# carpedkm/disentangled-subject-to-vid

Hardware: AMD Instinct MI355X
Metric: denoise steps/sec (CogVideoX-5B, 49f 720x480; one step = CFG-pair transformer forward + CFG + scheduler step) (higher is better)
Workload: dtype bf16

## Files before the change

### disentangled-subject-to-vid_amd/csrc/elementwise.hip

```cpp
#define S2V_HOST
#include "common.h"
#include "kernels.h"
#include <cstdlib>
#include <type_traits>

#define LN_MAX_FLOATS 64
template <typename T, int NR>
__device__ __forceinline__ void row_load(const T* x, int D, int lane, float* v) {
    constexpr int VN = Vec16<T>::N;
    const int chunks = D / VN;
#pragma unroll
    for (int i = 0; i < NR; ++i) {
        const int c = lane + 64 * i;
        const bool ok = c < chunks;
        Vec16<T>::ld(x + (ok ? c : 0) * VN, v + i * VN);
#pragma unroll
        for (int e = 0; e < VN; ++e) v[i * VN + e] = ok ? v[i * VN + e] : 0.f;
    }
}
template <typename T, int NR>
__device__ __forceinline__ void row_layernorm(float* v, int D, int lane, const T* w, const T* b, float eps) {
    constexpr int VN = Vec16<T>::N;
    const int chunks = D / VN;
    float s = 0.f;
#pragma unroll
    for (int i = 0; i < NR * VN; ++i) s += v[i];
    const float mean = wave_sum(s) / (float)D;
    float q = 0.f;
#pragma unroll
    for (int i = 0; i < NR; ++i) {
        const bool ok = lane + 64 * i < chunks;
#pragma unroll
        for (int e = 0; e < VN; ++e) {
            const float d = v[i * VN + e] - mean;
            q += ok ? d * d : 0.f;
        }
    }
    const float var = wave_sum(q) / (float)D;
    const float rstd = 1.0f / sqrtf(var + eps);
#pragma unroll
    for (int i = 0; i < NR; ++i) {
        const int c = lane + 64 * i;
        const bool ok = c < chunks;
        const int cc = ok ? c : 0;
        float wv[VN], bv[VN];
        Vec16<T>::ld(w + cc * VN, wv);
        Vec16<T>::ld(b + cc * VN, bv);
#pragma unroll
        for (int e = 0; e < VN; ++e) v[i * VN + e] = ok ? ET<T>::rnd((v[i * VN + e] - mean) * rstd * wv[e] + bv[e]) : 0.f;
    }
}
template <typename T, int NR>
__device__ __forceinline__ void row_modulate_store(float* v, int D, int lane, const T* shift, const T* scale, T* y) {
    constexpr int VN = Vec16<T>::N;
    const int chunks = D / VN;
#pragma unroll
    for (int i = 0; i < NR; ++i) {
        const int c = lane + 64 * i;
        const bool ok = c < chunks;
        const int cc = ok ? c : 0;
        float sc[VN], sh[VN], o[VN];
        Vec16<T>::ld(scale + cc * VN, sc);
        Vec16<T>::ld(shift + cc * VN, sh);
#pragma unroll
        for (int e = 0; e < VN; ++e) {
            const float s1 = ET<T>::rnd(1.0f + sc[e]);
            const float p = ET<T>::rnd(v[i * VN + e] * s1);
            o[e] = p + sh[e];
        }
        if (ok) Vec16<T>::st(y + c * VN, o);
    }
}
template <int NR>
__device__ __forceinline__ void row_modulate_quant_store(float* v, int D, int lane, const bf16_t* shift, const bf16_t* scale, unsigned char* q,
                                                         float* qscale, bf16_t* y = nullptr ) {
    const int chunks = D / 8;
    float amax = 0.f;
#pragma unroll
    for (int i = 0; i < NR; ++i) {
        const int c = lane + 64 * i;
        const bool ok = c < chunks;
        const int cc = ok ? c : 0;
        float sc[8], sh[8];
        Vec16<bf16_t>::ld(scale + cc * 8, sc);
        Vec16<bf16_t>::ld(shift + cc * 8, sh);
#pragma unroll
        for (int e = 0; e < 8; ++e) {
            const float s1 = ET<bf16_t>::rnd(1.0f + sc[e]);
            const float p = ET<bf16_t>::rnd(v[i * 8 + e] * s1);
            const float o = ok ? ET<bf16_t>::rnd(p + sh[e]) : 0.f;
            v[i * 8 + e] = o;
            amax = fmaxf(amax, fabsf(o));
        }
    }
    amax = wave_max(amax);
    const float sc = amax > 0.f ? amax * (1.0f / 448.0f) : 1.0f;
    const float inv = 1.0f / sc;
    if (lane == 0) *qscale = sc;
#pragma unroll
    for (int i = 0; i < NR; ++i) {
        const int c = lane + 64 * i;
        int w0 = 0, w1 = 0;
        w0 = __builtin_amdgcn_cvt_pk_fp8_f32(v[i * 8 + 0] * inv, v[i * 8 + 1] * inv, w0, false);
        w0 = __builtin_amdgcn_cvt_pk_fp8_f32(v[i * 8 + 2] * inv, v[i * 8 + 3] * inv, w0, true);
        w1 = __builtin_amdgcn_cvt_pk_fp8_f32(v[i * 8 + 4] * inv, v[i * 8 + 5] * inv, w1, false);
        w1 = __builtin_amdgcn_cvt_pk_fp8_f32(v[i * 8 + 6] * inv, v[i * 8 + 7] * inv, w1, true);
        if (c < chunks) *(u32x2*)(q + c * 8) = u32x2{(unsigned)w0, (unsigned)w1};
        if (y != nullptr && c < chunks) Vec16<bf16_t>::st(y + c * 8, v + i * 8);
    }
}
template <typename T, int NR>
struct RowParams { typename Vec16<T>::raw_t w[NR], b[NR], sc[NR], sh[NR]; };
template <typename T, int NR>
__device__ __forceinline__ void row_params(RowParams<T, NR>& p, int D, int lane, const T* w, const T* b, const T* scale, const T* shift) {
    constexpr int VN = Vec16<T>::N;
    const int chunks = D / VN;
#pragma unroll
    for (int i = 0; i < NR; ++i) {
        const int c = lane + 64 * i;
        const int cc = c < chunks ? c : 0;
        p.w[i] = Vec16<T>::ldraw(w + cc * VN);
        p.b[i] = Vec16<T>::ldraw(b + cc * VN);
        p.sc[i] = Vec16<T>::ldraw(scale + cc * VN);
        p.sh[i] = Vec16<T>::ldraw(shift + cc * VN);
    }
    __builtin_amdgcn_sched_barrier(0);
}
template <typename T, int NR>
__device__ __forceinline__ void row_layernorm_p(float* v, int D, int lane, const RowParams<T, NR>& p, float eps) {
    constexpr int VN = Vec16<T>::N;
    const int chunks = D / VN;
    float s = 0.f;
#pragma unroll
    for (int i = 0; i < NR * VN; ++i) s += v[i];
    const float mean = wave_sum(s) / (float)D;
    float q = 0.f;
#pragma unroll
    for (int i = 0; i < NR; ++i) {
        const bool ok = lane + 64 * i < chunks;
#pragma unroll
        for (int e = 0; e < VN; ++e) {
            const float d = v[i * VN + e] - mean;
            q += ok ? d * d : 0.f;
        }
    }
    const float var = wave_sum(q) / (float)D;
    const float rstd = 1.0f / sqrtf(var + eps);
#pragma unroll
    for (int i = 0; i < NR; ++i) {
        const bool ok = lane + 64 * i < chunks;
        float wv[VN], bv[VN];
        Vec16<T>::dec(p.w[i], wv);
        Vec16<T>::dec(p.b[i], bv);
#pragma unroll
        for (int e = 0; e < VN; ++e) v[i * VN + e] = ok ? ET<T>::rnd((v[i * VN + e] - mean) * rstd * wv[e] + bv[e]) : 0.f;
    }
}
template <typename T, int NR>
__device__ __forceinline__ void row_modulate_store_p(float* v, int D, int lane, const RowParams<T, NR>& p, T* y) {
    constexpr int VN = Vec16<T>::N;
    const int chunks = D / VN;
#pragma unroll
    for (int i = 0; i < NR; ++i) {
        const int c = lane + 64 * i;
        float sc[VN], sh[VN], o[VN];
        Vec16<T>::dec(p.sc[i], sc);
        Vec16<T>::dec(p.sh[i], sh);
#pragma unroll
        for (int e = 0; e < VN; ++e) {
            const float s1 = ET<T>::rnd(1.0f + sc[e]);
            const float pr = ET<T>::rnd(v[i * VN + e] * s1);
            o[e] = pr + sh[e];
        }
        if (c < chunks) Vec16<T>::st(y + c * VN, o);
    }
}

template <typename T> static int ln_rounds(int D) {
    const int need = (D / Vec16<T>::N + 63) / 64;
    for (int r : {1, 2, 3, 4, 6, 8, 12, 16})
        if (r >= need) return r;
    return -1;
}
#define S2V_LN_DISPATCH(T, D, ...)                                                   \
    switch (ln_rounds<T>(D)) {                                                        \
        case 1: { constexpr int NR = 1; __VA_ARGS__; } break;                                \
        case 2: { constexpr int NR = 2; __VA_ARGS__; } break;                                \
        case 3: { constexpr int NR = 3; __VA_ARGS__; } break;                                \
        case 4: { constexpr int NR = 4; __VA_ARGS__; } break;                                \
        case 6: { constexpr int NR = 6; __VA_ARGS__; } break;                                \
        case 8: { constexpr int NR = 8; __VA_ARGS__; } break;                                \
        case 12: if constexpr (sizeof(T) == 4) { constexpr int NR = 12; __VA_ARGS__; } break; \
        case 16: if constexpr (sizeof(T) == 4) { constexpr int NR = 16; __VA_ARGS__; } break; \
        default: return s2v_fail(__FILE__, __LINE__, "layer norm: row too long", -1); \
    }

template <typename T, int NR>
__global__ __launch_bounds__(256) void ln_modulate_k(const LnModArgs a) {
    const int lane = threadIdx.x & 63;
    const int row = blockIdx.x * 4 + (threadIdx.x >> 6);
    if (row >= a.B * a.Ntok) return;
    const int b = row / a.Ntok, r = row - b * a.Ntok;
    const bool txt = r < a.text_len;
    const bool ref = a.shift_ref != nullptr && !txt && r < a.text_len + a.ref_len;
    const T* shift = (const T*)(txt ? a.shift_txt : ref ? a.shift_ref : a.shift_vid) + (size_t)b * a.mod_stride;
    const T* scale = (const T*)(txt ? a.scale_txt : ref ? a.scale_ref : a.scale_vid) + (size_t)b * a.mod_stride;
    float v[NR * Vec16<T>::N];
    if constexpr (std::is_same<T, bf16_t>::value) {
        if (a.q8 != nullptr) {
            row_load<T, NR>((const T*)a.x + (size_t)row * a.ldx, a.D, lane, v);
            row_layernorm<T, NR>(v, a.D, lane, (const T*)a.w, (const T*)a.b, a.eps);
            row_modulate_quant_store<NR>(v, a.D, lane, shift, scale, (unsigned char*)a.q8 + (size_t)row * a.D, a.q8_scale + row,
                                         a.q8_keep_y ? (bf16_t*)a.y + (size_t)row * a.ldy : nullptr);
            return;
        }
    }
    typename Vec16<T>::raw_t xr[NR];
    {
        constexpr int VN = Vec16<T>::N;
        const int chunks = a.D / VN;
        const T* x = (const T*)a.x + (size_t)row * a.ldx;
#pragma unroll
        for (int i = 0; i < NR; ++i) xr[i] = Vec16<T>::ldraw(x + (lane + 64 * i < chunks ? lane + 64 * i : 0) * VN);
        RowParams<T, NR> prm;
        row_params<T, NR>(prm, a.D, lane, (const T*)a.w, (const T*)a.b, scale, shift);
#pragma unroll
        for (int i = 0; i < NR; ++i) {
            Vec16<T>::dec(xr[i], v + i * VN);
            const bool ok = lane + 64 * i < chunks;
#pragma unroll
            for (int e = 0; e < VN; ++e) v[i * VN + e] = ok ? v[i * VN + e] : 0.f;
        }
        row_layernorm_p<T, NR>(v, a.D, lane, prm, a.eps);
        row_modulate_store_p<T, NR>(v, a.D, lane, prm, (T*)a.y + (size_t)row * a.ldy);
    }
}
template <typename T, int NR, int RPW>
__global__ __launch_bounds__(256) void ln_modulate_lds_k(const LnModArgs a) {
    extern __shared__ __attribute__((aligned(16))) char ln_smem[];
    constexpr int VN = Vec16<T>::N;
    const int lane = threadIdx.x & 63, wave = threadIdx.x >> 6;
    const int rows = a.B * a.Ntok, r0 = blockIdx.x * (4 * RPW), rl = min(r0 + 4 * RPW, rows) - 1;
    auto params_of = [&](int row, const T*& shift, const T*& scale) {
        const int b = row / a.Ntok, r = row - b * a.Ntok;
        const bool txt = r < a.text_len;
        const bool ref = a.shift_ref != nullptr && !txt && r < a.text_len + a.ref_len;
        shift = (const T*)(txt ? a.shift_txt : ref ? a.shift_ref : a.shift_vid) + (size_t)b * a.mod_stride;
        scale = (const T*)(txt ? a.scale_txt : ref ? a.scale_ref : a.scale_vid) + (size_t)b * a.mod_stride;
    };
    const T *sh0, *sc0, *sh1, *sc1;
    params_of(r0, sh0, sc0);
    params_of(rl, sh1, sc1);
    const bool uniform = sh0 == sh1 && sc0 == sc1;
    T* lw = (T*)ln_smem;
    T *lb = lw + a.D, *lsc = lb + a.D, *lsh = lsc + a.D;
    if (uniform) {
        const int chunks = a.D / VN;
        for (int c = threadIdx.x; c < chunks; c += 256) {
            *(typename Vec16<T>::raw_t*)(lw + c * VN) = Vec16<T>::ldraw((const T*)a.w + c * VN);
            *(typename Vec16<T>::raw_t*)(lb + c * VN) = Vec16<T>::ldraw((const T*)a.b + c * VN);
            *(typename Vec16<T>::raw_t*)(lsc + c * VN) = Vec16<T>::ldraw(sc0 + c * VN);
            *(typename Vec16<T>::raw_t*)(lsh + c * VN) = Vec16<T>::ldraw(sh0 + c * VN);
        }
        __syncthreads();
    }
#pragma unroll 1
    for (int k = 0; k < RPW; ++k) {
        const int row = r0 + k * 4 + wave;
        if (row >= rows) break;
        const T *pw = lw, *pb = lb, *psc = lsc, *psh = lsh;
        if (!uniform) { pw = (const T*)a.w; pb = (const T*)a.b; params_of(row, psh, psc); }
        float v[NR * VN];
        row_load<T, NR>((const T*)a.x + (size_t)row * a.ldx, a.D, lane, v);
        row_layernorm<T, NR>(v, a.D, lane, pw, pb, a.eps);
        if constexpr (std::is_same<T, bf16_t>::value) {
            if (a.q8 != nullptr) {
                row_modulate_quant_store<NR>(v, a.D, lane, psh, psc, (unsigned char*)a.q8 + (size_t)row * a.D, a.q8_scale + row,
                                             a.q8_keep_y ? (bf16_t*)a.y + (size_t)row * a.ldy : nullptr);
                continue;
            }
        }
        row_modulate_store<T, NR>(v, a.D, lane, psh, psc, (T*)a.y + (size_t)row * a.ldy);
    }
}
int launch_ln_modulate(const LnModArgs& a, int dtype, hipStream_t st) {
    S2V_REQUIRE(a.D <= 4096 && a.D % 8 == 0, "ln_modulate: D must be <= 4096 and a multiple of 8");
    S2V_REQUIRE(a.q8 == nullptr || (dtype == S2V_BF16 && a.q8_scale != nullptr), "ln_modulate: the fp8 output needs bf16 rows and a scale vector");
    const int rows = a.B * a.Ntok;
    dim3 grid((rows + 3) / 4);
    int lds_rows = 16384;
#ifdef S2V_DIAG
    if (const char* e = getenv("S2V_LN_LDS_ROWS")) lds_rows = atoi(e);
#endif
    if (dtype == S2V_BF16 && lds_rows > 0 && rows >= lds_rows) {
        constexpr int RPW = 4;
        dim3 g16((rows + 4 * RPW - 1) / (4 * RPW));
        const size_t lds = (size_t)4 * a.D * 2;
        S2V_LN_DISPATCH(bf16_t, a.D, hipLaunchKernelGGL((ln_modulate_lds_k<bf16_t, NR, RPW>), g16, dim3(256), lds, st, a))
        S2V_CHECK_HIP(hipGetLastError());
        return 0;
    }
    if (dtype == S2V_BF16) {
        S2V_LN_DISPATCH(bf16_t, a.D, hipLaunchKernelGGL((ln_modulate_k<bf16_t, NR>), grid, dim3(256), 0, st, a))
    } else if (dtype == S2V_F16) {
        S2V_LN_DISPATCH(f16_t, a.D, hipLaunchKernelGGL((ln_modulate_k<f16_t, NR>), grid, dim3(256), 0, st, a))
    } else {
        S2V_LN_DISPATCH(float, a.D, hipLaunchKernelGGL((ln_modulate_k<float, NR>), grid, dim3(256), 0, st, a))
    }
    S2V_CHECK_HIP(hipGetLastError());
    return 0;
}

template <typename T, int NR>
__global__ __launch_bounds__(256) void tail_norm_k(const TailNormArgs a) {
    const int lane = threadIdx.x & 63;
    const int idx = blockIdx.x * 4 + (threadIdx.x >> 6);
    if (idx >= a.B * a.V) return;
    const int b = idx / a.V, vr = idx - b * a.V;
    const size_t xrow = (size_t)b * a.Ntok + a.row0 + vr;
    float v[NR * Vec16<T>::N];
    row_load<T, NR>((const T*)a.x + xrow * a.ldx, a.D, lane, v);
    row_layernorm<T, NR>(v, a.D, lane, (const T*)a.w1, (const T*)a.b1, a.eps);
    row_layernorm<T, NR>(v, a.D, lane, (const T*)a.w2, (const T*)a.b2, a.eps);
    const T* shift = (const T*)a.shift + (size_t)b * a.mod_stride;
    const T* scale = (const T*)a.scale + (size_t)b * a.mod_stride;
    row_modulate_store<T, NR>(v, a.D, lane, shift, scale, (T*)a.y + (size_t)idx * a.ldy);
}
int launch_tail_norm(const TailNormArgs& a, int dtype, hipStream_t st) {
    S2V_REQUIRE(a.D <= 4096 && a.D % 8 == 0, "tail_norm: D must be <= 4096 and a multiple of 8");
    dim3 grid((a.B * a.V + 3) / 4);
    if (dtype == S2V_BF16) {
        S2V_LN_DISPATCH(bf16_t, a.D, hipLaunchKernelGGL((tail_norm_k<bf16_t, NR>), grid, dim3(256), 0, st, a))
    } else if (dtype == S2V_F16) {
        S2V_LN_DISPATCH(f16_t, a.D, hipLaunchKernelGGL((tail_norm_k<f16_t, NR>), grid, dim3(256), 0, st, a))
    } else {
        S2V_LN_DISPATCH(float, a.D, hipLaunchKernelGGL((tail_norm_k<float, NR>), grid, dim3(256), 0, st, a))
    }
    S2V_CHECK_HIP(hipGetLastError());
    return 0;
}

template <typename T>
__global__ __launch_bounds__(256) void qk_norm_rope_k(const QkNormRopeArgs a) {
    const int D = a.H * 64;
    const int row = blockIdx.x;
    const int t = blockIdx.y * 256 + threadIdx.x;
    if (t >= 2 * a.H * 8) return;
    const int which = t >= a.H * 8;
    const int hh = (t >> 3) - which * a.H;
    const int oct = t & 7;
    T* p = (T*)a.qkv + (size_t)row * a.ld_qkv + which * D + hh * 64 + oct * 8;
    const int r = row % a.Ntok;
    const bool rope = a.cos != nullptr && r >= a.text_len;
    const size_t tab = (size_t)(rope ? r - a.text_len : 0) * 64 + oct * 8;
    float v[8], cs[8], sn[8], wv[8], bv[8];
    if constexpr (sizeof(T) == 2) {
        Vec16<T>::ld(p, v);
    } else {
        Vec16<T>::ld(p, v);
        Vec16<T>::ld(p + 4, v + 4);
    }
    if (a.cos != nullptr) {
        Vec16<float>::ld(a.cos + tab, cs);
        Vec16<float>::ld(a.cos + tab + 4, cs + 4);
        Vec16<float>::ld(a.sin + tab, sn);
        Vec16<float>::ld(a.sin + tab + 4, sn + 4);
    }
    const T* w = (const T*)(which ? a.nk_w : a.nq_w) + oct * 8;
    const T* bb = (const T*)(which ? a.nk_b : a.nq_b) + oct * 8;
    if constexpr (sizeof(T) == 2) {
        Vec16<T>::ld(w, wv);
        Vec16<T>::ld(bb, bv);
    } else {
        Vec16<T>::ld(w, wv);
        Vec16<T>::ld(w + 4, wv + 4);
        Vec16<T>::ld(bb, bv);
        Vec16<T>::ld(bb + 4, bv + 4);
    }
    float s = 0.f;
#pragma unroll
    for (int e = 0; e < 8; ++e) s += v[e];
    s += __shfl_xor(s, 1, 64); s += __shfl_xor(s, 2, 64); s += __shfl_xor(s, 4, 64);
    const float mean = s * (1.0f / 64.0f);
    float q = 0.f;
#pragma unroll
    for (int e = 0; e < 8; ++e) { const float d = v[e] - mean; q += d * d; }
    q += __shfl_xor(q, 1, 64); q += __shfl_xor(q, 2, 64); q += __shfl_xor(q, 4, 64);
    const float rstd = 1.0f / sqrtf(q * (1.0f / 64.0f) + a.eps);
#pragma unroll
    for (int e = 0; e < 8; ++e) v[e] = ET<T>::rnd((v[e] - mean) * rstd * wv[e] + bv[e]);
    if (rope) {
#pragma unroll
        for (int e = 0; e < 8; e += 2) {
            const float x0 = v[e], x1 = v[e + 1];
            v[e] = ET<T>::rnd(x0 * cs[e] + (-x1) * sn[e]);
            v[e + 1] = ET<T>::rnd(x1 * cs[e + 1] + x0 * sn[e + 1]);
        }
    }
    if constexpr (sizeof(T) == 2) {
        Vec16<T>::st(p, v);
    } else {
        Vec16<T>::st(p, v);
        Vec16<T>::st(p + 4, v + 4);
    }
}

__global__ __launch_bounds__(256) void v_amax_k(const bf16_t* qkv, int ld_qkv, int H, int Ntok, unsigned* vamax) {
    const int n0 = blockIdx.x * 64, h = blockIdx.y, b = blockIdx.z;
    const int D = H * 64;
    unsigned m = 0;
    for (int i = threadIdx.x; i < 64 * 8; i += 256) {
        const int n = n0 + (i >> 3), cc = (i & 7) * 8;
        if (n < Ntok) {
            const u32x4 val = *(const u32x4*)(qkv + (size_t)(b * Ntok + n) * ld_qkv + 2 * D + h * 64 + cc);
#pragma unroll
            for (int e = 0; e < 4; ++e) m = max(m, max(val[e] & 0x7fffu, (val[e] >> 16) & 0x7fffu));
        }
    }
#pragma unroll
    for (int o = 32; o > 0; o >>= 1) m = max(m, (unsigned)__shfl_xor((int)m, o, 64));
    if ((threadIdx.x & 63) == 0 && m != 0) atomicMax(vamax + b * H + h, m);
}
__global__ __launch_bounds__(256) void v_transpose_k(const bf16_t* qkv, int ld_qkv, int B, int H, int Ntok, bf16_t* vt,
                                                     int ntok_pad, const unsigned* vamax) {
    __shared__ bf16_t tile[64][64 + 2];
    const int n0 = blockIdx.x * 64, h = blockIdx.y, b = blockIdx.z;
    const int D = H * 64;
    const int tid = threadIdx.x;
    const bool to_f16 = vamax != nullptr;
    const float vscale = to_f16 ? __uint_as_float((unsigned)(127 + vt_f16_shift(vamax[b * H + h])) << 23) : 1.0f;
    for (int i = tid; i < 64 * 8; i += 256) {
        const int rr = i >> 3, cc = (i & 7) * 8;
        const int n = n0 + rr;
        u32x4 val = {0, 0, 0, 0};
        if (n < Ntok) val = *(const u32x4*)(qkv + (size_t)(b * Ntok + n) * ld_qkv + 2 * D + h * 64 + cc);
#pragma unroll
        for (int e = 0; e < 4; ++e) {
            tile[rr][cc + 2 * e] = (bf16_t)(val[e] & 0xffff);
            tile[rr][cc + 2 * e + 1] = (bf16_t)(val[e] >> 16);
        }
    }
    __syncthreads();
    bf16_t* dst = vt + (size_t)(b * H + h) * 64 * ntok_pad;
    for (int i = tid; i < 64 * 64; i += 256) {
        const int d = i >> 6, pos = i & 63;
        const int tok = (pos & ~12) | ((pos & 4) << 1) | ((pos & 8) >> 1);
        if (n0 + tok < Ntok) {
            bf16_t v = tile[tok][d];
            if (to_f16) {
                float f = __uint_as_float((unsigned)v << 16) * vscale;
                f = f != f ? f : fminf(fmaxf(f, -65504.0f), 65504.0f);
                v = __builtin_bit_cast(unsigned short, (_Float16)f);
            }
            dst[(size_t)d * ntok_pad + n0 + pos] = v;
        }
        else if (n0 + pos < ntok_pad) dst[(size_t)d * ntok_pad + n0 + pos] = 0;
    }
}

__global__ __launch_bounds__(256) void qk_quant_mx_k(const bf16_t* qkv, int ld_qkv, int H, int Ntok, int ntok_pad, float q_prescale,
                                                      unsigned char* q8, unsigned short* q8s, unsigned char* k8, unsigned* k8s) {
    const int tile = blockIdx.x, h = blockIdx.y, b = blockIdx.z >> 1, is_k = blockIdx.z & 1;
    const int tid = threadIdx.x, kr = tid >> 2, qt = tid & 3, blk = qt >> 1;
    const int n = tile * 64 + kr;
    if (!is_k && n >= Ntok) return;
    const int D = H * 64;
    float x[16];
    if (n < Ntok) {
        const bf16_t* src = qkv + (size_t)(b * Ntok + n) * ld_qkv + is_k * D + h * 64 + qt * 16;
        const u32x4 v0 = *(const u32x4*)src, v1 = *(const u32x4*)(src + 8);
        const float c = is_k ? 1.0f : q_prescale;
#pragma unroll
        for (int e = 0; e < 4; ++e) {
            x[2 * e] = __uint_as_float(v0[e] << 16) * c; x[2 * e + 1] = __uint_as_float(v0[e] & 0xffff0000u) * c;
            x[8 + 2 * e] = __uint_as_float(v1[e] << 16) * c; x[8 + 2 * e + 1] = __uint_as_float(v1[e] & 0xffff0000u) * c;
        }
    } else {
#pragma unroll
        for (int e = 0; e < 16; ++e) x[e] = 0.f;
    }
    float amax = 0.f;
#pragma unroll
    for (int e = 0; e < 16; ++e) amax = fmaxf(amax, fabsf(x[e]));
    amax = fmaxf(amax, __shfl_xor(amax, 1, 64));
    unsigned eb = (__float_as_uint(amax * (1.0f / 448.0f)) + 0x7fffffu) >> 23;
    eb = n < Ntok ? min(max(eb, 1u), 253u) : 127u;
    const float inv = __uint_as_float((254u - eb) << 23);
    u32x4 o;
#pragma unroll
    for (int w = 0; w < 4; ++w) {
        int r = 0;
        r = __builtin_amdgcn_cvt_pk_fp8_f32(x[4 * w] * inv, x[4 * w + 1] * inv, r, false);
        r = __builtin_amdgcn_cvt_pk_fp8_f32(x[4 * w + 2] * inv, x[4 * w + 3] * inv, r, true);
        o[w] = (unsigned)r;
    }
    const size_t bh = (size_t)b * H + h;
    if (is_k) {
        *(u32x4*)(k8 + (bh * ntok_pad + n) * 64 + qt * 16) = o;
        if ((qt & 1) == 0)
            ((unsigned char*)k8s)[((bh * (ntok_pad / 64) + tile) * 64 + blk * 32 + (kr & 31)) * 4 + (kr >> 5)] = (unsigned char)eb;
    } else {
        *(u32x4*)(q8 + (bh * Ntok + n) * 64 + qt * 16) = o;
        if ((qt & 1) == 0) ((unsigned char*)q8s)[(bh * Ntok + n) * 2 + blk] = (unsigned char)eb;
    }
}
int launch_qk_quant_mx(const void* qkv, int ld_qkv, int B, int H, int Ntok, int ntok_pad, float q_prescale, unsigned char* q8, unsigned short* q8s,
                       unsigned char* k8, unsigned* k8s, hipStream_t st) {
    S2V_REQUIRE(ntok_pad % 64 == 0 && ntok_pad >= Ntok, "qk_quant_mx: ntok_pad must be a multiple of 64 covering Ntok");
    hipLaunchKernelGGL(qk_quant_mx_k, dim3(ntok_pad / 64, H, 2 * B), dim3(256), 0, st, (const bf16_t*)qkv, ld_qkv, H, Ntok, ntok_pad, q_prescale, q8,
                       q8s, k8, k8s);
    S2V_CHECK_HIP(hipGetLastError());
    return 0;
}

__global__ __launch_bounds__(256) void qk_norm_quant_mx_k(const QkNormRopeArgs a, float q_prescale, unsigned char* q8, unsigned short* q8s, unsigned char* k8,
                                                           unsigned* k8s, int hg) {
    const int tile = blockIdx.x, h0 = blockIdx.y * hg, b = blockIdx.z >> 1, is_k = blockIdx.z & 1;
    const int tid = threadIdx.x, kr = tid >> 2, qt = tid & 3, blk = qt >> 1;
    const int n = tile * 64 + kr;
    const int H = a.H, Ntok = a.Ntok, ntok_pad = a.ntok_pad;
    if (!is_k && n >= Ntok) return;
    const int D = H * 64;
    const bool live = n < Ntok;
    const bool rope = live && a.cos != nullptr && n >= a.text_len;
    float cs[16], sn[16], wv[16], bv[16];
    if (live) {
        const size_t tab = (size_t)(rope ? n - a.text_len : 0) * 64 + qt * 16;
        if (a.cos != nullptr) {
#pragma unroll
            for (int e = 0; e < 16; e += 4) {
                Vec16<float>::ld(a.cos + tab + e, cs + e);
                Vec16<float>::ld(a.sin + tab + e, sn + e);
            }
        }
        const bf16_t* w = (const bf16_t*)(is_k ? a.nk_w : a.nq_w) + qt * 16;
        const bf16_t* bb = (const bf16_t*)(is_k ? a.nk_b : a.nq_b) + qt * 16;
        Vec16<bf16_t>::ld(w, wv); Vec16<bf16_t>::ld(w + 8, wv + 8);
        Vec16<bf16_t>::ld(bb, bv); Vec16<bf16_t>::ld(bb + 8, bv + 8);
    }
    const float c = is_k ? 1.0f : q_prescale;
#pragma unroll 1
    for (int h = h0; h < h0 + hg; ++h) {
        float x[16];
        if (live) {
            const bf16_t* src = (const bf16_t*)a.qkv + (size_t)(b * Ntok + n) * a.ld_qkv + is_k * D + h * 64 + qt * 16;
            Vec16<bf16_t>::ld(src, x);
            Vec16<bf16_t>::ld(src + 8, x + 8);
            float s0 = 0.f, s1 = 0.f;
#pragma unroll
            for (int e = 0; e < 8; ++e) { s0 += x[e]; s1 += x[8 + e]; }
            float s = s0 + s1;
            s += __shfl_xor(s, 1, 64); s += __shfl_xor(s, 2, 64);
            const float mean = s * (1.0f / 64.0f);
            float q0 = 0.f, q1 = 0.f;
#pragma unroll
            for (int e = 0; e < 8; ++e) {
                const float d0 = x[e] - mean, d1 = x[8 + e] - mean;
                q0 += d0 * d0; q1 += d1 * d1;
            }
            float q = q0 + q1;
            q += __shfl_xor(q, 1, 64); q += __shfl_xor(q, 2, 64);
            const float rstd = 1.0f / sqrtf(q * (1.0f / 64.0f) + a.eps);
#pragma unroll
            for (int e = 0; e < 16; ++e) x[e] = ET<bf16_t>::rnd((x[e] - mean) * rstd * wv[e] + bv[e]);
            if (rope) {
#pragma unroll
                for (int e = 0; e < 16; e += 2) {
                    const float x0 = x[e], x1 = x[e + 1];
                    x[e] = ET<bf16_t>::rnd(x0 * cs[e] + (-x1) * sn[e]);
                    x[e + 1] = ET<bf16_t>::rnd(x1 * cs[e + 1] + x0 * sn[e + 1]);
                }
            }
#pragma unroll
            for (int e = 0; e < 16; ++e) x[e] *= c;
        } else {
#pragma unroll
            for (int e = 0; e < 16; ++e) x[e] = 0.f;
        }
        float amax = 0.f;
#pragma unroll
        for (int e = 0; e < 16; ++e) amax = fmaxf(amax, fabsf(x[e]));
        amax = fmaxf(amax, __shfl_xor(amax, 1, 64));
        unsigned eb = (__float_as_uint(amax * (1.0f / 448.0f)) + 0x7fffffu) >> 23;
        eb = live ? min(max(eb, 1u), 253u) : 127u;
        const float inv = __uint_as_float((254u - eb) << 23);
        u32x4 o;
#pragma unroll
        for (int w = 0; w < 4; ++w) {
            int r = 0;
            r = __builtin_amdgcn_cvt_pk_fp8_f32(x[4 * w] * inv, x[4 * w + 1] * inv, r, false);
            r = __builtin_amdgcn_cvt_pk_fp8_f32(x[4 * w + 2] * inv, x[4 * w + 3] * inv, r, true);
            o[w] = (unsigned)r;
        }
        const size_t bh = (size_t)b * H + h;
        if (is_k) {
            *(u32x4*)(k8 + (bh * ntok_pad + n) * 64 + qt * 16) = o;
            if ((qt & 1) == 0)
                ((unsigned char*)k8s)[((bh * (ntok_pad / 64) + tile) * 64 + blk * 32 + (kr & 31)) * 4 + (kr >> 5)] = (unsigned char)eb;
        } else {
            *(u32x4*)(q8 + (bh * Ntok + n) * 64 + qt * 16) = o;
            if ((qt & 1) == 0) ((unsigned char*)q8s)[(bh * Ntok + n) * 2 + blk] = (unsigned char)eb;
        }
    }
}
int launch_qk_norm_quant_mx(const QkNormRopeArgs& a, float q_prescale, unsigned char* q8, unsigned short* q8s, unsigned char* k8, unsigned* k8s, hipStream_t st) {
    S2V_REQUIRE(a.ntok_pad % 64 == 0 && a.ntok_pad >= a.Ntok, "qk_norm_quant_mx: ntok_pad must be a multiple of 64 covering Ntok");
    S2V_REQUIRE(a.nq_w && a.nq_b && a.nk_w && a.nk_b && (a.cos == nullptr) == (a.sin == nullptr), "qk_norm_quant_mx: LayerNorm parameters / rotary tables");
    const int hg = a.H % 4 == 0 ? 4 : a.H % 2 == 0 ? 2 : 1;
    hipLaunchKernelGGL(qk_norm_quant_mx_k, dim3(a.ntok_pad / 64, a.H / hg, 2 * a.B), dim3(256), 0, st, a, q_prescale, q8, q8s, k8, k8s, hg);
    S2V_CHECK_HIP(hipGetLastError());
    return 0;
}

int launch_qk_norm_rope(const QkNormRopeArgs& a, int dtype, hipStream_t st) {
// ... 374 lines not shown
```

### disentangled-subject-to-vid_amd/csrc/gemm_epi.h

```cpp
#pragma once
#include "common.h"
#include "kernels.h"
#include <type_traits>

#pragma clang fp contract(off)

template <typename T, int EPI>
__device__ __forceinline__ void epilogue4(const GemmArgs& a, int m, int n, const float v[4]) {
    if (m >= a.M) return;
    const T* bias = (const T*)a.bias;
    float y[4];
#pragma unroll
    for (int i = 0; i < 4; ++i) {
        float bv = (bias && n + i < a.N) ? ET<T>::ld(bias + n + i) : 0.f;
        y[i] = ET<T>::rnd(v[i] + bv);
    }
    if (EPI == EPI_BIAS_GELU) {
#pragma unroll
        for (int i = 0; i < 4; ++i) y[i] = ET<T>::rnd(gelu_tanh_f(y[i]));
    }
    if (EPI == EPI_BIAS_GATE_RES) {
        const int b = m / a.tok_per_batch;
        const int r = m - b * a.tok_per_batch;
        const void* gsel = r < a.text_len ? a.gate_txt : (a.gate_ref != nullptr && r < a.text_len + a.ref_len) ? a.gate_ref : a.gate_vid;
        const T* gate = (const T*)gsel + (size_t)b * a.gate_stride;
        T* x = (T*)a.X + (size_t)m * a.ldx + n;
#pragma unroll
        for (int i = 0; i < 4; ++i) {
            if (n + i < a.N) {
                float t = ET<T>::rnd(ET<T>::ld(gate + n + i) * y[i]);
                ET<T>::st(x + i, ET<T>::ld(x + i) + t);
            }
        }
        return;
    }
    if (EPI == EPI_BIAS_ADD) {
        const T* r = (const T*)a.R + (size_t)m * a.ldr + n;
#pragma unroll
        for (int i = 0; i < 4; ++i)
            if (n + i < a.N) y[i] = y[i] + ET<T>::ld(r + i);
    }
    T* c = (T*)a.C + (size_t)m * a.ldc + n;
    if (n + 3 < a.N && (a.ldc & 3) == 0) {
        if constexpr (std::is_same<T, bf16_t>::value) {
            u32x2 p;
            p.x = pack2bf(y[0], y[1]);
            p.y = pack2bf(y[2], y[3]);
            *(u32x2*)c = p;
        } else if constexpr (std::is_same<T, f16_t>::value) {
            u32x2 p;
            p.x = pack2h(y[0], y[1]);
            p.y = pack2h(y[2], y[3]);
            *(u32x2*)c = p;
        } else {
            *(f32x4*)c = (f32x4){y[0], y[1], y[2], y[3]};
        }
    } else {
#pragma unroll
        for (int i = 0; i < 4; ++i)
            if (n + i < a.N) ET<T>::st(c + i, y[i]);
    }
}

__device__ __forceinline__ float oct_sum(float v) {
    v += __int_as_float(__builtin_amdgcn_update_dpp(0, __float_as_int(v), 0xB1, 0xf, 0xf, true));
    v += __int_as_float(__builtin_amdgcn_update_dpp(0, __float_as_int(v), 0x4E, 0xf, 0xf, true));
    v += __int_as_float(__builtin_amdgcn_update_dpp(0, __float_as_int(v), 0x141, 0xf, 0xf, true));
    return v;
}

__device__ __forceinline__ void load_bias64(const GemmArgs& a, int nw, int hi, u32x2 (&bvec)[8]) {
    const bf16_t* bias = (const bf16_t*)a.bias;
    if (bias && nw + 64 <= a.N) {
#pragma unroll
        for (int q = 0; q < 8; ++q) bvec[q] = *(const u32x2*)(bias + nw + (q >> 2) * 32 + 8 * (q & 3) + 4 * hi);
    } else {
#pragma unroll
        for (int q = 0; q < 8; ++q) {
            const int nl = (q >> 2) * 32 + 8 * (q & 3) + 4 * hi;
            unsigned short t[4] = {0, 0, 0, 0};
#pragma unroll
            for (int e = 0; e < 4; ++e)
                if (bias && nw + nl + e < a.N) t[e] = ((const unsigned short*)bias)[nw + nl + e];
            bvec[q] = u32x2{(unsigned)t[0] | ((unsigned)t[1] << 16), (unsigned)t[2] | ((unsigned)t[3] << 16)};
        }
    }
}

template <typename T16> struct H2;
template <> struct H2<bf16_t> {
    static __device__ __forceinline__ float lo(unsigned w) { return __uint_as_float(w << 16); }
    static __device__ __forceinline__ float hi(unsigned w) { return __uint_as_float(w & 0xffff0000u); }
    static __device__ __forceinline__ unsigned pack(float a, float b) { return pack2bf(a, b); }
    static __device__ __forceinline__ float rnd(float v) { return bf2f(f2bf(v)); }
};
template <> struct H2<f16_t> {
    static __device__ __forceinline__ float lo(unsigned w) { return (float)__builtin_bit_cast(f16x2_t, w)[0]; }
    static __device__ __forceinline__ float hi(unsigned w) { return (float)__builtin_bit_cast(f16x2_t, w)[1]; }
    static __device__ __forceinline__ unsigned pack(float a, float b) { return pack2h(a, b); }
    static __device__ __forceinline__ float rnd(float v) { return (float)(f16_t)v; }
};
template <int EPI, int MB, bool SC = false, int GRP = 4, typename T16 = bf16_t>
__device__ __forceinline__ void epilogue_wave_b(const GemmArgs& a, const f32x16 (&acc)[2][MB], int mw, int nw, char* patch, int lane,
                                                const u32x2 (&bvec)[8]) {
    const int fr = lane & 31, hi = lane >> 5;
    const int c16 = lane & 7;
    const bool qk_head = EPI == EPI_BIAS_QKNORM && nw < 2 * a.qk_D;
    const bool qk_rot = qk_head && a.qk_cs != nullptr;
    float qw[8], qb[8];
    f32x4 rc[2][GRP], rs[2][GRP];
    bool rope[2][GRP];
    auto rot_load = [&](int it0, int buf) {
        const float inv_tok = 1.0f / (float)a.tok_per_batch;
#pragma unroll
        for (int u = 0; u < GRP; ++u) {
            const int m = min(mw + (it0 + u) * 8 + (lane >> 3), a.M - 1);
            int b = (int)((float)m * inv_tok);
            int r = m - b * a.tok_per_batch;
            if (r < 0) r += a.tok_per_batch;
            if (r >= a.tok_per_batch) r -= a.tok_per_batch;
            rope[buf][u] = qk_rot && r >= a.text_len;
            const float* tp = a.qk_cs + (size_t)(rope[buf][u] ? r - a.text_len : 0) * 64 + c16 * 4;
            if (qk_rot) {
                rc[buf][u] = *(const f32x4*)tp;
                rs[buf][u] = *(const f32x4*)(tp + 32);
            }
        }
    };
    if (EPI == EPI_BIAS_QKNORM) {
        const int which = nw >= a.qk_D;
        const u32x4 w4 = *(const u32x4*)((const bf16_t*)a.qk_w[which] + c16 * 8), b4 = *(const u32x4*)((const bf16_t*)a.qk_b[which] + c16 * 8);
#pragma unroll
        for (int e = 0; e < 4; ++e) {
            qw[2 * e] = H2<T16>::lo(w4[e]); qw[2 * e + 1] = H2<T16>::hi(w4[e]);
            qb[2 * e] = H2<T16>::lo(b4[e]); qb[2 * e + 1] = H2<T16>::hi(b4[e]);
        }
        rot_load(0, 0);
    }
    constexpr bool PRE = EPI == EPI_BIAS_ADD && MB == 2;
    u32x4 xpre[PRE ? MB * 4 : 1];
    if (PRE) {
        const int npre = nw + c16 * 8 < a.N ? nw + c16 * 8 : 0;
#pragma unroll
        for (int it = 0; it < MB * 4; ++it)
            xpre[it] = *(const u32x4*)((const bf16_t*)a.R + (size_t)min(mw + it * 8 + (lane >> 3), a.M - 1) * a.ldr + npre);
        __builtin_amdgcn_sched_barrier(0);
    }
    float sa[MB];
#pragma unroll
    for (int j = 0; j < MB; ++j) sa[j] = (SC && a.a_scale) ? a.a_scale[min(mw + j * 32 + fr, a.M - 1)] : 1.f;
#pragma unroll
    for (int i = 0; i < 2; ++i)
#pragma unroll
        for (int rq = 0; rq < 4; ++rq) {
            const int nl = i * 32 + 8 * rq + 4 * hi;
            const u32x2 bq = bvec[i * 4 + rq];
            f32x4 sw = {1.f, 1.f, 1.f, 1.f};
            if (SC) sw = *(const f32x4*)(a.w_scale + nw + nl);
            const float bv[4] = {H2<T16>::lo(bq.x), H2<T16>::hi(bq.x), H2<T16>::lo(bq.y),
                                 H2<T16>::hi(bq.y)};
#pragma unroll
            for (int j = 0; j < MB; ++j) {
                float y[4];
#pragma unroll
                for (int e = 0; e < 4; ++e) y[e] = (SC ? acc[i][j][rq * 4 + e] * (sa[j] * sw[e]) : acc[i][j][rq * 4 + e]) + bv[e];
                const int row = j * 32 + fr;
                u32x2 p;
                p.x = H2<T16>::pack(y[0], y[1]);
                p.y = H2<T16>::pack(y[2], y[3]);
                if (EPI == EPI_BIAS_GELU) {
                    p.x = H2<T16>::pack(gelu_tanh_fast(H2<T16>::lo(p.x)), gelu_tanh_fast(H2<T16>::hi(p.x)));
                    p.y = H2<T16>::pack(gelu_tanh_fast(H2<T16>::lo(p.y)), gelu_tanh_fast(H2<T16>::hi(p.y)));
                }
                *(u32x2*)(patch + row * 128 + ((((nl >> 3) ^ (row & 7))) << 4) + (nl & 4) * 2) = p;
            }
        }
    const int n = nw + c16 * 8;
    const bool n_ok = n < a.N;
    const int nc = n_ok ? n : 0;
#pragma unroll
    for (int it0 = 0; it0 < MB * 4; it0 += GRP) {
        u32x4 v[GRP], g[GRP], xo[GRP];
        int mrow[GRP];
        const int cur = (it0 / GRP) & 1;
        if (EPI == EPI_BIAS_QKNORM && it0 + GRP < MB * 4) rot_load(it0 + GRP, cur ^ 1);
#pragma unroll
        for (int u = 0; u < GRP; ++u) {
            const int row = (it0 + u) * 8 + (lane >> 3);
            mrow[u] = mw + row;
            v[u] = *(const u32x4*)(patch + row * 128 + ((c16 ^ (row & 7)) << 4));
            const int m = min(mrow[u], a.M - 1);
            if (EPI == EPI_BIAS_GATE_RES) {
                const int b = m / a.tok_per_batch;
                const int r = m - b * a.tok_per_batch;
                const void* gsel = r < a.text_len ? a.gate_txt : (a.gate_ref != nullptr && r < a.text_len + a.ref_len) ? a.gate_ref : a.gate_vid;
                g[u] = *(const u32x4*)((const bf16_t*)gsel + (size_t)b * a.gate_stride + nc);
                xo[u] = *(const u32x4*)((const bf16_t*)a.X + (size_t)m * a.ldx + nc);
            } else if (EPI == EPI_BIAS_ADD) {
                if (PRE) xo[u] = xpre[PRE ? it0 + u : 0];
                else xo[u] = *(const u32x4*)((const bf16_t*)a.R + (size_t)m * a.ldr + nc);
            }
        }
#pragma unroll
        for (int u = 0; u < GRP; ++u) {
            u32x4 o = v[u];
            if (EPI == EPI_BIAS_QKNORM && qk_head) {
                float x[8];
#pragma unroll
                for (int e = 0; e < 4; ++e) { x[2 * e] = H2<T16>::lo(v[u][e]); x[2 * e + 1] = H2<T16>::hi(v[u][e]); }
                float s = 0.f;
#pragma unroll
                for (int e = 0; e < 8; ++e) s += x[e];
                s = oct_sum(s);
                const float mean = s * (1.0f / 64.0f);
                float q = 0.f;
#pragma unroll
                for (int e = 0; e < 8; ++e) { const float d = x[e] - mean; q += d * d; }
                q = oct_sum(q);
                const float rstd = 1.0f / sqrtf(q * (1.0f / 64.0f) + a.qk_eps);
#pragma unroll
                for (int e = 0; e < 8; ++e) x[e] = H2<T16>::rnd(((x[e] - mean) * rstd * qw[e] + qb[e]));
                if (rope[cur][u]) {
#pragma unroll
                    for (int e = 0; e < 8; e += 2) {
                        const float x0 = x[e], x1 = x[e + 1];
                        const float cc = rc[cur][u][e >> 1], ss = rs[cur][u][e >> 1];
                        x[e] = H2<T16>::rnd((x0 * cc + (-x1) * ss));
                        x[e + 1] = H2<T16>::rnd((x1 * cc + x0 * ss));
                    }
                }
#pragma unroll
                for (int e = 0; e < 4; ++e) o[e] = H2<T16>::pack(x[2 * e], x[2 * e + 1]);
            }
            if (EPI == EPI_BIAS_GATE_RES) {
#pragma unroll
                for (int e = 0; e < 4; ++e) {
                    const float t0 = H2<T16>::rnd((H2<T16>::lo(g[u][e]) * H2<T16>::lo(v[u][e])));
                    const float t1 = H2<T16>::rnd((H2<T16>::hi(g[u][e]) * H2<T16>::hi(v[u][e])));
                    o[e] = H2<T16>::pack(H2<T16>::lo(xo[u][e]) + t0, H2<T16>::hi(xo[u][e]) + t1);
                }
            } else if (EPI == EPI_BIAS_ADD) {
#pragma unroll
                for (int e = 0; e < 4; ++e)
                    o[e] = H2<T16>::pack(H2<T16>::lo(v[u][e]) + H2<T16>::lo(xo[u][e]),
                                   H2<T16>::hi(v[u][e]) + H2<T16>::hi(xo[u][e]));
            }
            if (EPI == EPI_BIAS_GELU && a.mx_out_q) {
                typedef unsigned short u16x2_t __attribute__((ext_vector_type(2)));
                u16x2_t pm = __builtin_bit_cast(u16x2_t, o[0] & 0x7fff7fffu);
#pragma unroll
                for (int e = 1; e < 4; ++e) pm = __builtin_elementwise_max(pm, __builtin_bit_cast(u16x2_t, o[e] & 0x7fff7fffu));
                int amb = (int)max((unsigned)pm[0], (unsigned)pm[1]) << 16;
                amb = max(amb, __builtin_amdgcn_update_dpp(0, amb, 0xB1, 0xf, 0xf, true));
                amb = max(amb, __builtin_amdgcn_update_dpp(0, amb, 0x4E, 0xf, 0xf, true));
                unsigned eb = (__float_as_uint(__int_as_float(amb) * (1.0f / 448.0f)) + 0x7fffffu) >> 23;
                eb = min(max(eb, 1u), 254u);
                const float bscale = __uint_as_float(eb << 23);
                unsigned w0 = 0, w1 = 0;
                asm volatile("v_cvt_scalef32_pk_fp8_bf16 %0, %1, %2" : "+v"(w0) : "v"(o[0]), "v"(bscale));
                asm volatile("v_cvt_scalef32_pk_fp8_bf16 %0, %1, %2 op_sel:[0,0,1]" : "+v"(w0) : "v"(o[1]), "v"(bscale));
                asm volatile("v_cvt_scalef32_pk_fp8_bf16 %0, %1, %2" : "+v"(w1) : "v"(o[2]), "v"(bscale));
                asm volatile("v_cvt_scalef32_pk_fp8_bf16 %0, %1, %2 op_sel:[0,0,1]" : "+v"(w1) : "v"(o[3]), "v"(bscale));
                const unsigned e2 = eb | ((unsigned)__builtin_amdgcn_update_dpp(0, (int)eb, 0x104, 0xf, 0xf, true) << 8);
                if (mrow[u] < a.M && n_ok) {
                    *(u32x2*)(a.mx_out_q + (size_t)mrow[u] * a.N + n) = u32x2{w0, w1};
                    if (c16 == 0) *(unsigned short*)(a.mx_out_s + ((size_t)(n >> 7) * a.mx_rows + mx_perm_row(mrow[u])) * 4 + ((n >> 5) & 3)) = (unsigned short)e2;
                }
            } else if (mrow[u] < a.M && n_ok) {
                if (EPI == EPI_BIAS_GATE_RES) *(u32x4*)((bf16_t*)a.X + (size_t)mrow[u] * a.ldx + n) = o;
                else *(u32x4*)((bf16_t*)a.C + (size_t)mrow[u] * a.ldc + n) = o;
            }
        }
    }
}
template <int EPI, int MB, bool SC = false, typename T16 = bf16_t>
__device__ __forceinline__ void epilogue_wave(const GemmArgs& a, const f32x16 (&acc)[2][MB], int mw, int nw, char* patch, int lane) {
    u32x2 bvec[8];
    load_bias64(a, nw, lane >> 5, bvec);
    epilogue_wave_b<EPI, MB, SC, 4, T16>(a, acc, mw, nw, patch, lane, bvec);
}
template <int MB>
__device__ __forceinline__ void lora_up_wave(const GemmArgs& a, f32x16 (&acc)[2][MB], int mw, int nw, int lane) {
    const int fr = lane & 31, hi = lane >> 5;
    float sa[MB];
#pragma unroll
    for (int j = 0; j < MB; ++j) sa[j] = a.a_scale ? a.a_scale[min(mw + j * 32 + fr, a.M - 1)] : 1.f;
#pragma unroll
    for (int i = 0; i < 2; ++i)
#pragma unroll
        for (int rq = 0; rq < 4; ++rq) {
            const f32x4 sw = *(const f32x4*)(a.w_scale + nw + i * 32 + 8 * rq + 4 * hi);
#pragma unroll
            for (int j = 0; j < MB; ++j)
#pragma unroll
                for (int e = 0; e < 4; ++e) acc[i][j][rq * 4 + e] = acc[i][j][rq * 4 + e] * (sa[j] * sw[e]);
        }
    const int seg = a.lora_seg > 0 ? min(nw, a.N - 1) / a.lora_seg : 0;
    const bf16_t* tp = (const bf16_t*)a.lora_t + (size_t)(mw + fr) * a.lora_ldt + seg * a.lora_r + 8 * hi;
    const bf16_t* bp = (const bf16_t*)a.lora_bs + (size_t)(nw + fr) * a.lora_r + 8 * hi;
    for (int k = 0; k < a.lora_r; k += 16) {
        bf16x8 bf[2], tf[MB];
#pragma unroll
        for (int i = 0; i < 2; ++i) bf[i] = *(const bf16x8*)(bp + (size_t)i * 32 * a.lora_r + k);
#pragma unroll
        for (int j = 0; j < MB; ++j) tf[j] = *(const bf16x8*)(tp + (size_t)j * 32 * a.lora_ldt + k);
#pragma unroll
        for (int i = 0; i < 2; ++i)
#pragma unroll
            for (int j = 0; j < MB; ++j) acc[i][j] = __builtin_amdgcn_mfma_f32_32x32x16_bf16(bf[i], tf[j], acc[i][j], 0, 0, 0);
    }
}
template <int EPI>
__device__ __forceinline__ void epilogue_wave64(const GemmArgs& a, const f32x16 (&acc)[2][2], int mw, int nw, char* patch,
                                                int lane) {
    epilogue_wave<EPI, 2>(a, acc, mw, nw, patch, lane);
}
__host__ __device__ __forceinline__ bool epi_vec_ok(const GemmArgs& a, int epi) {
    if ((a.N & 7) != 0) return false;
    if (epi == EPI_BIAS_GATE_RES) return (a.ldx & 7) == 0 && (a.gate_stride & 7) == 0;
    if (epi == EPI_BIAS_ADD && (a.ldr & 7) != 0) return false;
    return (a.ldc & 7) == 0;
}


#ifdef S2V_TU_FP_CONTRACT_OFF
#pragma clang fp contract(off)
#else
#pragma clang fp contract(fast)
#endif
```

Before: 1.586.

## Prefetch next row in LN-modulate and hoist residual/gate loads in gated-residual epilogue

The LDS-based LN-modulate kernel now issues the next row's global loads before running layernorm on the current row, so memory latency overlaps compute. The gated-residual GEMM epilogue loads residual X rows up front (all at once, or double-buffered in groups) and computes the gate index once per tile using a float-reciprocal division. When a tile lies within a single batch/segment it uses one gate vector, otherwise it re-fetches the gate only when the segment changes. A diagnostic entry point for LN-modulate is also added under S2V_DIAG. The cost is higher register pressure and more code paths in the epilogue.

```diff
diff --git a/disentangled-subject-to-vid_amd/csrc/elementwise.hip b/disentangled-subject-to-vid_amd/csrc/elementwise.hip
--- a/disentangled-subject-to-vid_amd/csrc/elementwise.hip
+++ b/disentangled-subject-to-vid_amd/csrc/elementwise.hip
@@ -264,6 +264,14 @@
         }
         __syncthreads();
     }
+    const int chunks = a.D / VN;
+    typename Vec16<T>::raw_t xr[NR];
+    auto request = [&](int row) {
+        const T* x = (const T*)a.x + (size_t)min(row, rows - 1) * a.ldx;
+#pragma unroll
+        for (int i = 0; i < NR; ++i) xr[i] = Vec16<T>::ldraw(x + (lane + 64 * i < chunks ? lane + 64 * i : 0) * VN);
+    };
+    request(r0 + wave);
 #pragma unroll 1
     for (int k = 0; k < RPW; ++k) {
         const int row = r0 + k * 4 + wave;
@@ -271,7 +279,15 @@
         const T *pw = lw, *pb = lb, *psc = lsc, *psh = lsh;
         if (!uniform) { pw = (const T*)a.w; pb = (const T*)a.b; params_of(row, psh, psc); }
         float v[NR * VN];
-        row_load<T, NR>((const T*)a.x + (size_t)row * a.ldx, a.D, lane, v);
+#pragma unroll
+        for (int i = 0; i < NR; ++i) {
+            Vec16<T>::dec(xr[i], v + i * VN);
+            const bool ok = lane + 64 * i < chunks;
+#pragma unroll
+            for (int e = 0; e < VN; ++e) v[i * VN + e] = ok ? v[i * VN + e] : 0.f;
+        }
+        if (k + 1 < RPW) request(row + 4);
+        __builtin_amdgcn_sched_barrier(0);
         row_layernorm<T, NR>(v, a.D, lane, pw, pb, a.eps);
         if constexpr (std::is_same<T, bf16_t>::value) {
             if (a.q8 != nullptr) {
@@ -310,6 +326,22 @@
     S2V_CHECK_HIP(hipGetLastError());
     return 0;
 }
+#ifdef S2V_DIAG
+extern "C" __attribute__((visibility("default"))) int s2v_diag_ln_modulate(const void* x, void* y, const void* w, const void* b, const void* mod,
+                                                                            int32_t mod_stride, int32_t B, int32_t Ntok, int32_t text_len, int32_t ref_len,
+                                                                            int32_t with_ref, int32_t D, float eps, void* q8, float* q8_scale, void* stream) {
+    S2V_REQUIRE(x && y && w && b && mod, "s2v_diag_ln_modulate: null argument");
+    const char* mb = (const char*)mod;
+    const int64_t E = 2;
+    LnModArgs n{};
+    n.x = x; n.ldx = D; n.y = y; n.ldy = D; n.w = w; n.b = b; n.eps = eps;
+    n.shift_vid = mb; n.scale_vid = mb + D * E; n.shift_txt = mb + 3 * D * E; n.scale_txt = mb + 4 * D * E;
+    n.mod_stride = mod_stride; n.B = B; n.Ntok = Ntok; n.text_len = text_len; n.D = D;
+    if (with_ref) { n.shift_ref = mb + 6 * D * E; n.scale_ref = mb + 7 * D * E; n.ref_len = ref_len; }
+    n.q8 = q8; n.q8_scale = q8_scale;
+    return launch_ln_modulate(n, S2V_BF16, (hipStream_t)stream);
+}
+#endif
 
 template <typename T, int NR>
 __global__ __launch_bounds__(256) void tail_norm_k(const TailNormArgs a) {
diff --git a/disentangled-subject-to-vid_amd/csrc/gemm_epi.h b/disentangled-subject-to-vid_amd/csrc/gemm_epi.h
--- a/disentangled-subject-to-vid_amd/csrc/gemm_epi.h
+++ b/disentangled-subject-to-vid_amd/csrc/gemm_epi.h
@@ -146,6 +146,47 @@
             xpre[it] = *(const u32x4*)((const bf16_t*)a.R + (size_t)min(mw + it * 8 + (lane >> 3), a.M - 1) * a.ldr + npre);
         __builtin_amdgcn_sched_barrier(0);
     }
+    constexpr bool GR = EPI == EPI_BIAS_GATE_RES;
+    constexpr int NG = MB * 4;
+    constexpr bool GR_ALL = MB <= 2 || !SC;
+    constexpr int XN = !GR ? 1 : GR_ALL ? NG : 2 * GRP;
+    u32x4 xres[XN], gcur;
+    int gr_b = 0, gr_seg = 0, gr_b0 = 0, gr_r0 = 0, gr_m0 = 0;
+    float gr_inv = 0.f;
+    bool gr_one = true;
+    const int gr_nc = nw + c16 * 8 < a.N ? nw + c16 * 8 : 0;
+    auto gr_row = [&](int it) { return min(mw + it * 8 + (lane >> 3), a.M - 1); };
+    auto gr_index = [&](int m, int& b, int& seg) {
+        const int x = gr_r0 + (m - gr_m0);
+        int q = (int)((float)x * gr_inv);
+        int r = (int)((unsigned)x - (unsigned)q * (unsigned)a.tok_per_batch);
+        if (r < 0) { r += a.tok_per_batch; --q; }
+        if (r >= a.tok_per_batch) { r -= a.tok_per_batch; ++q; }
+        b = gr_b0 + q;
+        seg = r < a.text_len ? 0 : (a.gate_ref != nullptr && r < a.text_len + a.ref_len) ? 1 : 2;
+    };
+    auto gr_gate = [&](int b, int seg) {
+        const void* gsel = seg == 0 ? a.gate_txt : seg == 1 ? a.gate_ref : a.gate_vid;
+        return *(const u32x4*)((const bf16_t*)gsel + (size_t)b * a.gate_stride + gr_nc);
+    };
+    auto gr_xload = [&](int it0, int cnt) {
+#pragma unroll
+        for (int u = 0; u < cnt; ++u) xres[(it0 + u) % XN] = *(const u32x4*)((const bf16_t*)a.X + (size_t)gr_row(it0 + u) * a.ldx + gr_nc);
+    };
+    if (GR) {
+        gr_xload(0, GR_ALL ? NG : GRP);
+        gr_m0 = min(mw, a.M - 1);
+        gr_b0 = gr_m0 / a.tok_per_batch;
+        gr_r0 = gr_m0 - gr_b0 * a.tok_per_batch;
+        gr_inv = 1.0f / (float)a.tok_per_batch;
+        int bl, sl;
+        gr_index(gr_m0, gr_b, gr_seg);
+        gr_index(min(mw + MB * 32 - 1, a.M - 1), bl, sl);
+        gr_one = __builtin_amdgcn_readfirstlane((int)(gr_b == bl && gr_seg == sl)) != 0;
+        gr_index(gr_row(0), gr_b, gr_seg);
+        gcur = gr_gate(gr_b, gr_seg);
+        __builtin_amdgcn_sched_barrier(0);
+    }
     float sa[MB];
 #pragma unroll
     for (int j = 0; j < MB; ++j) sa[j] = (SC && a.a_scale) ? a.a_scale[min(mw + j * 32 + fr, a.M - 1)] : 1.f;
@@ -179,24 +220,23 @@
     const bool n_ok = n < a.N;
     const int nc = n_ok ? n : 0;
 #pragma unroll
+    for (int pass = 0; pass < (GR ? 2 : 1); ++pass) {
+    const bool one_gate = pass == 0;
+    if (GR && gr_one != one_gate) continue;
+#pragma unroll
     for (int it0 = 0; it0 < MB * 4; it0 += GRP) {
-        u32x4 v[GRP], g[GRP], xo[GRP];
+        u32x4 v[GRP], xo[GRP];
         int mrow[GRP];
         const int cur = (it0 / GRP) & 1;
         if (EPI == EPI_BIAS_QKNORM && it0 + GRP < MB * 4) rot_load(it0 + GRP, cur ^ 1);
+        if (GR && !GR_ALL && it0 + GRP < NG) gr_xload(it0 + GRP, GRP);
 #pragma unroll
         for (int u = 0; u < GRP; ++u) {
             const int row = (it0 + u) * 8 + (lane >> 3);
             mrow[u] = mw + row;
             v[u] = *(const u32x4*)(patch + row * 128 + ((c16 ^ (row & 7)) << 4));
             const int m = min(mrow[u], a.M - 1);
-            if (EPI == EPI_BIAS_GATE_RES) {
-                const int b = m / a.tok_per_batch;
-                const int r = m - b * a.tok_per_batch;
-                const void* gsel = r < a.text_len ? a.gate_txt : (a.gate_ref != nullptr && r < a.text_len + a.ref_len) ? a.gate_ref : a.gate_vid;
-                g[u] = *(const u32x4*)((const bf16_t*)gsel + (size_t)b * a.gate_stride + nc);
-                xo[u] = *(const u32x4*)((const bf16_t*)a.X + (size_t)m * a.ldx + nc);
-            } else if (EPI == EPI_BIAS_ADD) {
+            if (EPI == EPI_BIAS_ADD) {
                 if (PRE) xo[u] = xpre[PRE ? it0 + u : 0];
                 else xo[u] = *(const u32x4*)((const bf16_t*)a.R + (size_t)m * a.ldr + nc);
             }
@@ -204,6 +244,15 @@
 #pragma unroll
         for (int u = 0; u < GRP; ++u) {
             u32x4 o = v[u];
+            if (GR) {
+                if (!one_gate && it0 + u > 0) {
+                    int b, seg;
+                    gr_index(gr_row(it0 + u), b, seg);
+                    if (b != gr_b || seg != gr_seg) gcur = gr_gate(b, seg);
+                    gr_b = b; gr_seg = seg;
+                }
+                xo[u] = xres[(it0 + u) % XN];
+            }
             if (EPI == EPI_BIAS_QKNORM && qk_head) {
                 float x[8];
 #pragma unroll
@@ -235,8 +284,8 @@
             if (EPI == EPI_BIAS_GATE_RES) {
 #pragma unroll
                 for (int e = 0; e < 4; ++e) {
-                    const float t0 = H2<T16>::rnd((H2<T16>::lo(g[u][e]) * H2<T16>::lo(v[u][e])));
-                    const float t1 = H2<T16>::rnd((H2<T16>::hi(g[u][e]) * H2<T16>::hi(v[u][e])));
+                    const float t0 = H2<T16>::rnd((H2<T16>::lo(gcur[e]) * H2<T16>::lo(v[u][e])));
+                    const float t1 = H2<T16>::rnd((H2<T16>::hi(gcur[e]) * H2<T16>::hi(v[u][e])));
                     o[e] = H2<T16>::pack(H2<T16>::lo(xo[u][e]) + t0, H2<T16>::hi(xo[u][e]) + t1);
                 }
             } else if (EPI == EPI_BIAS_ADD) {
@@ -272,6 +321,7 @@
             }
         }
     }
+    }
 }
 template <int EPI, int MB, bool SC = false, typename T16 = bf16_t>
 __device__ __forceinline__ void epilogue_wave(const GemmArgs& a, const f32x16 (&acc)[2][MB], int mw, int nw, char* patch, int lane) {
```

After: 1.594, median of 2. Within noise of the previous version (+0.5%).
